# bg5sbk/dragonboat

Hardware: AMD Instinct MI355X
Metric: quorum-commit decisions/sec (whole node) + % HBM roofline at 1/2/4/8 GPUs (higher is better)
Workload: dtype u64

## Files before the change

### dragonboat_amd/csrc/hq_commit_body.h

```cpp
#pragma once

#include <type_traits>

#include "hq_internal.h"

namespace {

typedef uint64_t u64x2 __attribute__((ext_vector_type(2)));
typedef uint32_t u32x4 __attribute__((ext_vector_type(4)));

__device__ __forceinline__ u64x2 ld_stream2(const uint64_t *p) {
    return __builtin_nontemporal_load(reinterpret_cast<const u64x2 *>(p));
}
__device__ __forceinline__ void st_stream2(uint64_t *p, u64x2 v) {
    *reinterpret_cast<u64x2 *>(p) = v;
}

struct CommitK {
    uint64_t G;
    uint64_t stride;
    const uint64_t *match;
    const uint64_t *cin;
    uint64_t *cout;
    const uint64_t *last;
    const void *aux;
    const void *ring;
    uint64_t *changed, *fallback;
    const uint8_t *nv;
    uint32_t R, reserved;
};
static_assert(sizeof(CommitK) == 96, "keep the decision kernels' argument at 96 bytes");

__device__ __forceinline__ void ce(uint64_t &a, uint64_t &b) {
    const uint64_t lo = a < b ? a : b;
    const uint64_t hi = a < b ? b : a;
    a = lo;
    b = hi;
}

template <int N>
__device__ __forceinline__ void sort_net(uint64_t (&v)[N]) {
#pragma unroll
    for (int r = 0; r < N; ++r) {
#pragma unroll
        for (int i = r & 1; i + 1 < N; i += 2) ce(v[i], v[i + 1]);
    }
}

template <int N>
__device__ __forceinline__ uint64_t quorum_match_uniform(uint64_t (&v)[N]) {
    if constexpr (N == 1) {
        return v[0];
    } else if constexpr (N == 2) {
        return v[0] < v[1] ? v[0] : v[1];
    } else if constexpr (N == 3) {
        ce(v[0], v[1]);
        ce(v[1], v[2]);
        return v[0] > v[1] ? v[0] : v[1];
    } else {
        sort_net<N>(v);
        return v[N - (N / 2 + 1)];
    }
}

template <int N>
__device__ __forceinline__ uint64_t quorum_match_pern(uint64_t (&v)[N], int n) {
    sort_net<N>(v);
    const int idx = N - (n / 2 + 1);
    uint64_t r = 0;
#pragma unroll
    for (int k = 0; k < N; ++k) r = (k == idx) ? v[k] : r;
    return r;
}

__device__ __forceinline__ uint64_t spread32(uint32_t x) {
    uint64_t v = x;
    v = (v | (v << 16)) & 0x0000FFFF0000FFFFull;
    v = (v | (v << 8)) & 0x00FF00FF00FF00FFull;
    v = (v | (v << 4)) & 0x0F0F0F0F0F0F0F0Full;
    v = (v | (v << 2)) & 0x3333333333333333ull;
    v = (v | (v << 1)) & 0x5555555555555555ull;
    return v;
}

template <int N, int FORM, bool PERN>
__device__ __forceinline__ void decide(const CommitK &a, uint64_t g, uint64_t (&m)[N], int n,
                                       uint64_t cin, uint64_t last, uint64_t aux,
                                       uint64_t &cout, bool &chg, bool &fb) {
    cout = cin;
    chg = false;
    fb = false;
    if constexpr (PERN) {
        if (n < 1 || n > N) {
            fb = true;
            return;
        }
#pragma unroll
        for (int s = 0; s < N; ++s) m[s] = (s < n) ? m[s] : 0;
    }
    uint64_t q;
    if constexpr (PERN) {
        q = quorum_match_pern<N>(m, n);
    } else {
        q = quorum_match_uniform<N>(m);
    }
    if constexpr (FORM == HQ_FORM_TERM_START) {
        chg = (q > cin) & (q >= aux) & (q <= last);
    } else if constexpr (FORM == HQ_FORM_TERM_MASK) {
        fb = (cin > last) || (last - cin > a.R);
        chg = !fb && q > cin && q <= last && ((aux >> (q & (uint64_t)(a.R - 1))) & 1);
    } else if constexpr (FORM == HQ_FORM_TERM_RING32) {
        fb = (aux == 0) | (aux >= 0xFFFFFFFFull) | (cin > last) || (last - cin > a.R);
        if (!fb && q > cin && q <= last) {
            const uint32_t lterm = static_cast<const uint32_t *>(a.ring)[g * a.R + (q & (uint64_t)(a.R - 1))];
            chg = lterm == (uint32_t)aux;
        }
    } else {
        fb = (aux == 0) | (cin > last) || (last - cin > a.R);
        if (!fb && q > cin && q <= last) {
            const uint64_t lterm = static_cast<const uint64_t *>(a.ring)[g * a.R + (q & (uint64_t)(a.R - 1))];
            chg = lterm == aux;
        }
    }
    cout = chg ? q : cin;
}

#ifndef HQ_TILE_SCHED_BARRIER
#define HQ_TILE_SCHED_BARRIER 1
#endif

template <bool WT>
__device__ __forceinline__ void st8(uint64_t *p, uint64_t v) {
    if constexpr (WT) __hip_atomic_store(p, v, __ATOMIC_RELAXED, __HIP_MEMORY_SCOPE_AGENT);
    else *p = v;
}

template <class T>
__device__ __forceinline__ T *byte_off(T *p, uint32_t off) {
    return reinterpret_cast<T *>(reinterpret_cast<
        typename std::conditional<std::is_const<T>::value, const char, char>::type *>(p) + off);
}

template <int N, int FORM, bool PERN, int LEAD, bool INPLACE, bool WT = false, bool SOFF = false>
__device__ __forceinline__ void commit_tile(const CommitK &a, uint64_t wbase, uint64_t lane) {
    constexpr uint64_t T = HQ_TILE_GROUPS, H = T / 2;
    constexpr int NR = N - LEAD;
    const uint64_t *t = a.match + (wbase / T) * a.stride + lane * 2;
    const uint64_t ga = wbase + lane, gb = ga + H;
    bool ca = false, cb = false, fa = false, fb = false;
    if (wbase + T <= a.G) {
        const uint64_t *tb = a.match + (wbase / T) * a.stride;
        const uint32_t lo = (uint32_t)lane * 16u;
        auto row = [&](int r) -> const uint64_t * {
            if constexpr (SOFF) return byte_off(tb + r * T, lo);
            return t + r * T;
        };
        uint64_t m0[N], m1[N];
#pragma unroll
        for (int s = LEAD; s < N; ++s) {
            const u64x2 v = ld_stream2(row(s - LEAD));
            m0[s] = v.x;
            m1[s] = v.y;
        }
        const u64x2 ci = ld_stream2(row(NR)), la = ld_stream2(row(NR + 1));
        if constexpr (LEAD) {
            m0[0] = la.x;
            m1[0] = la.y;
        }
        u64x2 ax;
        if constexpr (FORM == HQ_FORM_TERM_MASK) {
            const uint32_t *mp =
                SOFF ? byte_off(reinterpret_cast<const uint32_t *>(tb + (NR + 2) * T), lo / 4)
                     : reinterpret_cast<const uint32_t *>(
                           reinterpret_cast<const uint16_t *>(t - lane * 2 + (NR + 2) * T) + lane * 2);
            const uint32_t mm = __builtin_nontemporal_load(mp);
            ax = (u64x2){mm & 0xFFFFu, mm >> 16};
        } else {
            ax = ld_stream2(row(NR + 2));
        }
#if HQ_TILE_SCHED_BARRIER
        if constexpr (N <= 5) __builtin_amdgcn_sched_barrier(0);
#endif
        const int na = PERN ? (int)a.nv[ga] : N, nb = PERN ? (int)a.nv[gb] : N;
        uint64_t coa, cob;
#ifdef HQ_TILE_COPY
        coa = ci.x ^ la.x ^ ax.x;
        cob = ci.y ^ la.y ^ ax.y;
#pragma unroll
        for (int s = LEAD; s < N; ++s) {
            coa ^= m0[s];
            cob ^= m1[s];
        }
        ca = coa & 1;
        cb = cob & 1;
        (void)na;
        (void)nb;
#else
        decide<N, FORM, PERN>(a, ga, m0, na, ci.x, la.x, ax.x, coa, ca, fa);
        decide<N, FORM, PERN>(a, gb, m1, nb, ci.y, la.y, ax.y, cob, cb, fb);
#endif
        if constexpr (INPLACE) {
            uint64_t *cr = const_cast<uint64_t *>(row(NR));
            if constexpr (WT) {
                st8<true>(cr, coa);
                st8<true>(cr + 1, cob);
            } else {
                st_stream2(cr, (u64x2){coa, cob});
            }
        } else if constexpr (SOFF) {
            uint64_t *cb0 = a.cout + wbase;
            st8<WT>(byte_off(cb0, lo / 2), coa);
            st8<WT>(byte_off(cb0 + H, lo / 2), cob);
        } else {
            st8<WT>(a.cout + ga, coa);
            st8<WT>(a.cout + gb, cob);
        }
    } else {
        auto single = [&](int j, bool &c, bool &f) {
            const uint64_t g = ga + H * j;
            uint64_t m[N];
            const uint64_t last = t[(NR + 1) * T + j];
#pragma unroll
            for (int s = LEAD; s < N; ++s) m[s] = t[(s - LEAD) * T + j];
            if constexpr (LEAD) m[0] = last;
            const uint64_t ax =
                FORM == HQ_FORM_TERM_MASK
                    ? (uint64_t)reinterpret_cast<const uint16_t *>(t - lane * 2 + (NR + 2) * T)[lane * 2 + j]
                    : t[(NR + 2) * T + j];
            uint64_t co;
            decide<N, FORM, PERN>(a, g, m, PERN ? (int)a.nv[g] : N, t[NR * T + j], last, ax,
                                  co, c, f);
            if constexpr (INPLACE) st8<WT>(const_cast<uint64_t *>(t) + NR * T + j, co);
            else st8<WT>(a.cout + g, co);
        };
        if (ga < a.G) single(0, ca, fa);
        if (gb < a.G) single(1, cb, fb);
    }
    const uint64_t ba = __ballot(ca), bb = __ballot(cb);
    const uint64_t xa = __ballot(fa), xb = __ballot(fb);
    const uint64_t w = (wbase >> 6) + lane;
    if (lane < 2 && w < ((a.G + 63) >> 6)) {
        if (a.changed) st8<WT>(a.changed + w, lane ? bb : ba);
        if (a.fallback) st8<WT>(a.fallback + w, lane ? xb : xa);
    }
}

}
```

### dragonboat_amd/csrc/hq_engine.hip

```cpp
#include <algorithm>
#include <chrono>
#include <cstdlib>
#include <cstring>
#include <mutex>
#include <new>
#include <string>
#include <thread>

#include "hq_commit_body.h"

namespace {

constexpr uint32_t kEngineMaxDepth = 64;
constexpr uint64_t kDescStop = 1;
constexpr int kShards = 8;
constexpr int kPollCopies = 16;
constexpr int kPollStride = 32;
constexpr int kInit = 32;

struct EngineDesc {
    uint64_t G;
    const uint64_t *tiles;
    uint64_t *cout;
    uint64_t *changed;
    uint64_t *fallback;
    uint64_t seq;
    uint64_t flags;
    uint64_t per;
};
static_assert(sizeof(EngineDesc) == 64, "a descriptor is 8 relay lanes of u64");

struct EngineK {
    uint64_t stride;
    uint64_t idle_ticks;
    uint32_t R;
    uint32_t depth;
    uint32_t signal;
    uint32_t epoch;
    const uint64_t *h_posted;
    uint64_t *h_done;
    uint64_t *h_clock;
    const EngineDesc *h_ring;
    uint64_t *d_posted;
    uint64_t *d_arrive;
    uint64_t *d_top;
    uint64_t *d_cursor;
    EngineDesc *d_ring;
    uint64_t *d_polled;
    uint64_t *d_exit;
    uint64_t init_base;
    uint32_t init_count, pad;
    EngineDesc init[kInit];
};

__device__ __forceinline__ uint64_t uniform64(uint64_t v) {
    const uint32_t lo = __builtin_amdgcn_readfirstlane((uint32_t)v);
    const uint32_t hi = __builtin_amdgcn_readfirstlane((uint32_t)(v >> 32));
    return ((uint64_t)hi << 32) | lo;
}

__device__ __forceinline__ uint64_t now_ticks() { return __builtin_amdgcn_s_memrealtime(); }

template <class T>
__device__ __forceinline__ T *as_global(uint64_t v) {
    typedef __attribute__((address_space(1))) T GT;
    return (T *)(GT *)v;
}

typedef __attribute__((address_space(1))) const volatile EngineK GlobalEngineK;
__device__ __forceinline__ GlobalEngineK &kargs() {
    return *(GlobalEngineK *)reinterpret_cast<uintptr_t>(__builtin_amdgcn_kernarg_segment_ptr());
}

template <class T>
__device__ __forceinline__ T *gp(T *p) { return as_global<T>(reinterpret_cast<uint64_t>(p)); }

__device__ void relay(GlobalEngineK &e, uint32_t lane) {
    const uint64_t have = __hip_atomic_load(gp(e.d_posted), __ATOMIC_RELAXED, __HIP_MEMORY_SCOPE_AGENT);
    const uint64_t hp = __hip_atomic_load(gp(e.h_posted), __ATOMIC_RELAXED, __HIP_MEMORY_SCOPE_SYSTEM);
    if (hp <= have) return;
    __builtin_amdgcn_fence(__ATOMIC_ACQUIRE, "");
    const uint64_t n = hp - have < e.depth ? hp - have : e.depth;
    const uint64_t dmask = e.depth - 1;
    for (uint64_t base = 0; base < n; base += 32) {
        uint64_t v[4];
#pragma unroll
        for (int j = 0; j < 4; ++j) {
            const uint64_t i = base + (lane >> 3) + 8 * j;
            v[j] = i < n ? __hip_atomic_load(
                               reinterpret_cast<const uint64_t *>(gp(e.h_ring) + ((have + i) & dmask)) +
                                   (lane & 7),
                               __ATOMIC_RELAXED, __HIP_MEMORY_SCOPE_SYSTEM)
                         : 0;
        }
#pragma unroll
        for (int j = 0; j < 4; ++j) {
            const uint64_t i = base + (lane >> 3) + 8 * j;
            if (i < n)
                __hip_atomic_store(reinterpret_cast<uint64_t *>(gp(e.d_ring) + ((have + i) & dmask)) +
                                       (lane & 7),
                                   v[j], __ATOMIC_RELAXED, __HIP_MEMORY_SCOPE_AGENT);
        }
    }
    __builtin_amdgcn_fence(__ATOMIC_RELEASE, "agent");
    if (lane == 0)
        __hip_atomic_store(gp(e.d_posted), have + n, __ATOMIC_RELAXED, __HIP_MEMORY_SCOPE_AGENT);
    if (lane < (uint32_t)kPollCopies)
        __hip_atomic_store(gp(e.d_polled) + lane * kPollStride, have + n, __ATOMIC_RELAXED,
                           __HIP_MEMORY_SCOPE_AGENT);
}

__device__ void arrive(GlobalEngineK &e, uint64_t s) {
    const uint64_t slot = s & (e.depth - 1);
    const uint32_t shard = blockIdx.x % kShards;
    const uint32_t nshard = gridDim.x < (uint32_t)kShards ? gridDim.x : (uint32_t)kShards;
    const uint64_t per = (gridDim.x - shard + kShards - 1) / kShards;
    uint64_t *ctr = gp(e.d_arrive) + slot * kShards + shard;
    if (__hip_atomic_fetch_add(ctr, (uint64_t)1, __ATOMIC_RELAXED, __HIP_MEMORY_SCOPE_AGENT) + 1 !=
        per)
        return;
    __hip_atomic_store(ctr, (uint64_t)0, __ATOMIC_RELAXED, __HIP_MEMORY_SCOPE_AGENT);
    if (__hip_atomic_fetch_add(gp(e.d_top) + slot, (uint64_t)1, __ATOMIC_RELAXED,
                               __HIP_MEMORY_SCOPE_AGENT) + 1 != nshard)
        return;
    __hip_atomic_store(gp(e.d_top) + slot, (uint64_t)0, __ATOMIC_RELAXED, __HIP_MEMORY_SCOPE_AGENT);
    __hip_atomic_store(gp(e.h_clock) + slot, now_ticks(), __ATOMIC_RELAXED, __HIP_MEMORY_SCOPE_SYSTEM);
    __hip_atomic_store(gp(e.h_done) + slot, s + 1, __ATOMIC_RELEASE, __HIP_MEMORY_SCOPE_SYSTEM);
}

struct EngineLds {
    EngineDesc ring[kEngineMaxDepth];
    uint32_t end[kEngineMaxDepth];
    uint32_t fin[kEngineMaxDepth];
    uint32_t tgt[kEngineMaxDepth];
    uint64_t known;
    uint32_t ticket;
    uint32_t top_end;
    uint32_t done;
    uint32_t waiting, lock, exit;
};

__device__ __forceinline__ bool before(uint32_t a, uint32_t b) { return (int32_t)(a - b) < 0; }

__device__ __forceinline__ uint64_t wg_len(uint64_t G, uint64_t per) {
    const uint64_t tiles = (G + HQ_TILE_GROUPS - 1) / HQ_TILE_GROUPS;
    const uint64_t b0 = (uint64_t)blockIdx.x * per;
    return b0 >= tiles ? 0 : (tiles - b0 < per ? tiles - b0 : per);
}

__device__ void install(GlobalEngineK &e, EngineLds &l, uint64_t from, uint64_t to) {
    const uint64_t dmask = e.depth - 1;
    uint32_t top = l.top_end;
    for (uint64_t s = from; s < to; ++s) {
        const EngineDesc &d = l.ring[s & dmask];
        const uint32_t len = (d.flags & kDescStop) ? 0u : (uint32_t)wg_len(d.G, d.per);
        top += len;
        l.end[s & dmask] = top;
        l.tgt[s & dmask] += len;
        if (len == 0 && e.signal && !(d.flags & kDescStop)) arrive(e, s);
    }
    l.top_end = top;
}

__device__ __forceinline__ uint64_t lds_known(EngineLds &l) {
    return __hip_atomic_load(&l.known, __ATOMIC_ACQUIRE, __HIP_MEMORY_SCOPE_WORKGROUP);
}

__device__ __forceinline__ uint32_t wave_u32(uint32_t v) { return __builtin_amdgcn_readfirstlane(v); }

__device__ __forceinline__ uint64_t polled(GlobalEngineK &e) {
    return uniform64(__hip_atomic_load(gp(e.d_polled) + (blockIdx.x % kPollCopies) * kPollStride,
                                       __ATOMIC_RELAXED, __HIP_MEMORY_SCOPE_AGENT));
}

__device__ __forceinline__ void pull(GlobalEngineK &e, EngineLds &l, uint64_t from, uint64_t p,
                                     uint32_t lane) {
    __builtin_amdgcn_fence(__ATOMIC_ACQUIRE, "agent");
    const uint64_t dmask = e.depth - 1;
    for (uint64_t i = lane >> 3; i < p - from; i += 8) {
        const uint64_t slot = (from + i) & dmask;
        reinterpret_cast<uint64_t *>(l.ring + slot)[lane & 7] = __hip_atomic_load(
            reinterpret_cast<const uint64_t *>(gp(e.d_ring) + slot) + (lane & 7),
            __ATOMIC_RELAXED, __HIP_MEMORY_SCOPE_AGENT);
    }
    if (lane == 0) {
        install(e, l, from, p);
        __hip_atomic_store(&l.known, p, __ATOMIC_RELEASE, __HIP_MEMORY_SCOPE_WORKGROUP);
    }
}

template <int WPW>
__device__ uint64_t frontier(GlobalEngineK &e, EngineLds &l, uint64_t s, uint32_t lane) {
    uint64_t k = lds_known(l);
    if (k > s) return k;
    const bool relayer = blockIdx.x == 0;
    if (lane == 0) __hip_atomic_fetch_add(&l.waiting, 1u, __ATOMIC_RELAXED, __HIP_MEMORY_SCOPE_WORKGROUP);
    for (;;) {
        k = uniform64(lds_known(l));
        if (k > s) break;
        if (wave_u32(__hip_atomic_load(&l.exit, __ATOMIC_RELAXED, __HIP_MEMORY_SCOPE_WORKGROUP)))
            return s;
        uint32_t got = 0;
        if (lane == 0)
            got = __hip_atomic_exchange(&l.lock, 1u, __ATOMIC_ACQUIRE, __HIP_MEMORY_SCOPE_WORKGROUP) == 0;
        if (wave_u32(got)) {
            k = uniform64(lds_known(l));
            if (k > s) {
                if (lane == 0) __hip_atomic_store(&l.lock, 0u, __ATOMIC_RELEASE, __HIP_MEMORY_SCOPE_WORKGROUP);
                break;
            }
            const uint64_t t0 = now_ticks();
            uint32_t backoff = 1;
            bool leave = false;
            for (;;) {
                if (relayer) relay(e, lane);
                const uint64_t p = polled(e);
                if (p > s) {
                    pull(e, l, s, p, lane);
                    k = p;
                    break;
                }
                const bool all_waiting =
                    wave_u32(__hip_atomic_load(&l.waiting, __ATOMIC_RELAXED,
                                               __HIP_MEMORY_SCOPE_WORKGROUP)) == (uint32_t)WPW;
                if (relayer) {
                    if (all_waiting && now_ticks() - t0 > e.idle_ticks) {
                        __builtin_amdgcn_fence(__ATOMIC_RELEASE, "agent");
                        if (lane == 0)
                            __hip_atomic_store(gp(e.d_exit), (uint64_t)e.epoch, __ATOMIC_RELAXED,
                                               __HIP_MEMORY_SCOPE_AGENT);
                        leave = true;
                    }
                } else if (all_waiting) {
                    const bool ended = uniform64(__hip_atomic_load(gp(e.d_exit), __ATOMIC_RELAXED,
                                                                   __HIP_MEMORY_SCOPE_AGENT)) == e.epoch;
                    __builtin_amdgcn_fence(__ATOMIC_ACQUIRE, "agent");
                    const uint64_t p2 = polled(e);
                    if ((ended && p2 <= s) || now_ticks() - t0 > 64 * e.idle_ticks) leave = true;
                }
                if (leave) {
                    if (lane == 0)
                        __hip_atomic_store(&l.exit, 1u, __ATOMIC_RELAXED, __HIP_MEMORY_SCOPE_WORKGROUP);
                    k = s;
                    break;
                }
                for (uint32_t i = 0; i < backoff; ++i) __builtin_amdgcn_s_sleep(16);
                backoff = backoff < 4 ? 2 * backoff : 4;
            }
            if (lane == 0) __hip_atomic_store(&l.lock, 0u, __ATOMIC_RELEASE, __HIP_MEMORY_SCOPE_WORKGROUP);
            if (k == s) return s;
            break;
        }
        __builtin_amdgcn_s_sleep(4);
    }
    if (lane == 0) __hip_atomic_fetch_sub(&l.waiting, 1u, __ATOMIC_RELAXED, __HIP_MEMORY_SCOPE_WORKGROUP);
    return k;
}

__device__ void refresh(GlobalEngineK &e, EngineLds &l, uint64_t s, uint32_t lane) {
    if (uniform64(lds_known(l)) > s + 1) return;
    uint32_t got = 0;
    if (lane == 0)
        got = __hip_atomic_exchange(&l.lock, 1u, __ATOMIC_ACQUIRE, __HIP_MEMORY_SCOPE_WORKGROUP) == 0;
    if (!wave_u32(got)) return;
    const uint64_t k = uniform64(lds_known(l));
    if (blockIdx.x == 0) relay(e, lane);
    const uint64_t p = polled(e);
    if (p > k) pull(e, l, k, p, lane);
    if (lane == 0) __hip_atomic_store(&l.lock, 0u, __ATOMIC_RELEASE, __HIP_MEMORY_SCOPE_WORKGROUP);
}

__device__ __forceinline__ uint32_t claim(EngineLds &l, uint32_t lane) {
    uint32_t t = 0;
    if (lane == 0) t = __hip_atomic_fetch_add(&l.ticket, 1u, __ATOMIC_RELAXED, __HIP_MEMORY_SCOPE_WORKGROUP);
    return wave_u32(t);
}

#ifdef HQ_ENGINE_WGPROF
constexpr uint32_t kWgProfMax = 2048;
__device__ uint64_t g_wgprof[kWgProfMax * 8];
#endif

template <int N, int FORM, int LEAD, bool INPLACE, int BLK, bool SIG>
__global__ __launch_bounds__(BLK) __attribute__((amdgpu_waves_per_eu(BLK >= 1024 ? 8 : 1, 8)))
void k_commit_engine(const EngineK e) {
    constexpr int WPW = BLK / 64;
    __shared__ EngineLds l;
    const uint32_t lane = threadIdx.x & 63;
    const uint32_t wv = __builtin_amdgcn_readfirstlane(threadIdx.x >> 6);
    const uint64_t dmask = e.depth - 1;
    const uint64_t s0 = uniform64(gp(e.d_cursor)[blockIdx.x]);
    for (uint32_t i = threadIdx.x; i < kEngineMaxDepth; i += BLK) {
        l.fin[i] = 0;
        l.tgt[i] = 0;
    }
    for (uint32_t i = threadIdx.x; i < e.init_count * 8; i += BLK)
        reinterpret_cast<uint64_t *>(l.ring + ((e.init_base + (i >> 3)) & dmask))[i & 7] =
            reinterpret_cast<const uint64_t *>(e.init)[i];
    __syncthreads();
    if (threadIdx.x == 0) {
        const uint64_t top = e.init_base + e.init_count;
        l.ticket = 0;
        l.done = 0;
        l.top_end = 0;
        l.waiting = l.lock = l.exit = 0;
        if (top > s0) install(kargs(), l, s0, top);
        l.known = top > s0 ? top : s0;
    }
    __syncthreads();
    if (blockIdx.x == 0 && wv == 0) refresh(kargs(), l, s0, lane);
    uint64_t s = s0;
    uint64_t known = s0;
    uint32_t e_prev = 0;
#ifdef HQ_ENGINE_WGPROF
    uint64_t *const prof = blockIdx.x < kWgProfMax ? g_wgprof + (size_t)blockIdx.x * 8 : nullptr;
    uint64_t p_busy = 0, p_tiles = 0, p_front = 0, p_nfront = 0, p_refr = 0;
    if (prof && threadIdx.x == 0) {
        __hip_atomic_store(prof + 0, now_ticks(), __ATOMIC_RELAXED, __HIP_MEMORY_SCOPE_AGENT);
        __hip_atomic_store(prof + 1, (uint64_t)__builtin_amdgcn_s_getreg((3 << 11) | 20),
                           __ATOMIC_RELAXED, __HIP_MEMORY_SCOPE_AGENT);
        __hip_atomic_store(prof + 2, (uint64_t)__builtin_amdgcn_s_getreg((31 << 11) | 4),
                           __ATOMIC_RELAXED, __HIP_MEMORY_SCOPE_AGENT);
    }
#endif
    uint32_t t = claim(l, lane);
    bool pend = false;
    uint64_t p_s = 0;
    uint32_t p_tgt = 0;
    auto count = [&]() {
        if constexpr (INPLACE) {
            if (lane == 0)
                __hip_atomic_fetch_add(&l.done, 1u, __ATOMIC_RELEASE, __HIP_MEMORY_SCOPE_WORKGROUP);
        }
        if constexpr (SIG) {
            uint32_t f = 0;
            if (lane == 0)
                f = __hip_atomic_fetch_add(&l.fin[p_s & dmask], 1u, __ATOMIC_RELAXED,
                                           __HIP_MEMORY_SCOPE_WORKGROUP) + 1;
            if (wave_u32(f) == p_tgt && lane == 0) arrive(kargs(), p_s);
        }
        pend = false;
    };
    auto drain = [&]() {
        if constexpr (SIG || INPLACE) {
            if (pend) {
                asm volatile("s_waitcnt vmcnt(0)" ::: "memory");
                count();
            }
        }
    };
    for (;;) {
        if (s >= known) {
            drain();
            #ifdef HQ_ENGINE_WGPROF
            const uint64_t p_f0 = now_ticks();
            #endif
            known = frontier<WPW>(kargs(), l, s, lane);
            #ifdef HQ_ENGINE_WGPROF
            p_front += now_ticks() - p_f0;
            ++p_nfront;
            #endif
            if (known <= s) break;
        }
        const uint64_t slot = s & dmask;
        const uint64_t *d = reinterpret_cast<const uint64_t *>(l.ring + slot);
        if (uniform64(d[6]) & kDescStop) {
            drain();
            if (t == e_prev && lane == 0) arrive(kargs(), s);
            ++s;
            break;
        }
        const uint32_t e_cur = wave_u32(l.end[slot]);
        if (before(t, e_cur)) {
            CommitK k{};
            k.stride = e.stride;
            k.R = e.R;
            k.G = uniform64(d[0]);
            k.match = as_global<const uint64_t>(uniform64(d[1]));
            k.cout = as_global<uint64_t>(uniform64(d[2]));
            k.changed = as_global<uint64_t>(uniform64(d[3]));
            k.fallback = as_global<uint64_t>(uniform64(d[4]));
            const uint64_t b0 = (uint64_t)blockIdx.x * uniform64(d[7]);
            uint32_t tgt = 0;
            if constexpr (SIG) tgt = wave_u32(l.tgt[slot]);
            if constexpr (INPLACE) {
                drain();
                while (before(wave_u32(__hip_atomic_load(&l.done, __ATOMIC_ACQUIRE,
                                                         __HIP_MEMORY_SCOPE_WORKGROUP)),
                              e_prev))
                    __builtin_amdgcn_s_sleep(2);
            }
#ifdef HQ_ENGINE_WGPROF
            const uint64_t p_t0 = now_ticks();
#endif
            do {
                const uint64_t wbase = uniform64((b0 + (uint32_t)(t - e_prev)) * HQ_TILE_GROUPS);
                uint32_t ln;
                asm volatile("v_mov_b32 %0, %1" : "=v"(ln) : "v"(lane));
                commit_tile<N, FORM, false, LEAD, INPLACE, SIG, true>(k, wbase, ln);
                if constexpr (SIG || INPLACE) {
                    asm volatile("" ::: "memory");
                    if (pend) count();
                    pend = true;
                    p_s = s;
                    p_tgt = tgt;
                }
#ifdef HQ_ENGINE_WGPROF
                ++p_tiles;
#endif
                t = claim(l, lane);
            } while (before(t, e_cur));
#ifdef HQ_ENGINE_WGPROF
            p_busy += now_ticks() - p_t0;
#endif
        }
        e_prev = e_cur;
        ++s;
        #ifdef HQ_ENGINE_WGPROF
        const uint64_t p_r0 = now_ticks();
        #endif
        if (wv == 0) refresh(kargs(), l, s, lane);
        #ifdef HQ_ENGINE_WGPROF
        if (wv == 0) p_refr += now_ticks() - p_r0;
        #endif
    }
    drain();
    if (lane == 0 && wv == 0) gp(e.d_cursor)[blockIdx.x] = s;
#ifdef HQ_ENGINE_WGPROF
    if (prof && lane == 0) {
        __hip_atomic_fetch_add(prof + 3, p_busy, __ATOMIC_RELAXED, __HIP_MEMORY_SCOPE_AGENT);
        __hip_atomic_fetch_add(prof + 4, p_tiles, __ATOMIC_RELAXED, __HIP_MEMORY_SCOPE_AGENT);
        __hip_atomic_fetch_max(prof + 5, now_ticks(), __ATOMIC_RELAXED, __HIP_MEMORY_SCOPE_AGENT);
        __hip_atomic_fetch_add(prof + 6, p_front | (p_nfront << 40), __ATOMIC_RELAXED,
                               __HIP_MEMORY_SCOPE_AGENT);
        __hip_atomic_fetch_add(prof + 7, p_refr, __ATOMIC_RELAXED, __HIP_MEMORY_SCOPE_AGENT);
    }
#endif
}

typedef void (*EngineKernel)(const EngineK);

template <int N, int FORM, int LEAD, bool INPLACE>
void engine_kernel_for(bool sig, EngineKernel *fn, int *blk) {
    constexpr int B = N <= 5 ? 1024 : 512;
    *fn = sig ? k_commit_engine<N, FORM, LEAD, INPLACE, B, true>
              : k_commit_engine<N, FORM, LEAD, INPLACE, B, false>;
    *blk = B;
}

template <int N>
int engine_kernel_n(uint32_t form, uint32_t layout, bool sig, EngineKernel *fn, int *blk) {
    const bool lead = (layout & 0xFFu) == HQ_LAYOUT_TILES_LEADER;
    const bool inplace = (layout & HQ_LAYOUT_IN_PLACE) != 0;
#define HQ_ENGINE_PICK(F)                                                                        \
    if (inplace) engine_kernel_for<N, F, 1, true>(sig, fn, blk);                                 \
    else if (lead) engine_kernel_for<N, F, 1, false>(sig, fn, blk);                              \
    else engine_kernel_for<N, F, 0, false>(sig, fn, blk);
    if (form == HQ_FORM_TERM_MASK) {
        HQ_ENGINE_PICK(HQ_FORM_TERM_MASK)
    } else {
        HQ_ENGINE_PICK(HQ_FORM_TERM_START)
    }
#undef HQ_ENGINE_PICK
    return HQ_OK;
}

int engine_kernel(uint32_t n, uint32_t form, uint32_t layout, bool sig, EngineKernel *fn, int *blk) {
    switch (n) {
    case 1: return engine_kernel_n<1>(form, layout, sig, fn, blk);
    case 2: return engine_kernel_n<2>(form, layout, sig, fn, blk);
    case 3: return engine_kernel_n<3>(form, layout, sig, fn, blk);
    case 4: return engine_kernel_n<4>(form, layout, sig, fn, blk);
    case 5: return engine_kernel_n<5>(form, layout, sig, fn, blk);
    case 6: return engine_kernel_n<6>(form, layout, sig, fn, blk);
    case 7: return engine_kernel_n<7>(form, layout, sig, fn, blk);
    default: return engine_kernel_n<8>(form, layout, sig, fn, blk);
    }
}

}

struct hq_engine {
    hq_ctx *ctx = nullptr;
    std::mutex mu;
    std::string err;
    hq_engine_config cfg{};
    hipStream_t stream = nullptr;
    hipEvent_t ev_start = nullptr, ev_end = nullptr;
    EngineKernel fn = nullptr;
    int block = 0;
    uint32_t grid = 0;
    EngineK k{};
    char *host = nullptr;
    char *dev = nullptr;
    uint64_t posted = 0;
    uint64_t completed = 0;
    bool running = false;
    uint64_t launches = 0;
    double launch_ms = 0.0;
    uint64_t relaunches = 0;
    uint32_t epoch = 0;
    uint64_t wait_limit_ms = 60000;
    size_t cur_off = 0, exit_off = 0, polled_off = 0;
    uint64_t inplace_G = 0;
};

namespace {

int efail(hq_engine *e, int code, const std::string &msg) {
    e->err = msg;
    return code;
}

int echeck(hq_engine *e, hipError_t r, const char *what) {
    if (r == hipSuccess) return HQ_OK;
    return efail(e, r == hipErrorOutOfMemory ? HQ_E_NOMEM : HQ_E_DEVICE,
                 std::string(what) + ": " + hipGetErrorString(r));
}

uint64_t host_load(const uint64_t *p) { return __atomic_load_n(p, __ATOMIC_ACQUIRE); }

int fold_if_ended(hq_engine *e, bool *ended) {
    *ended = !e->running;
    if (!e->running) return HQ_OK;
    const hipError_t q = hipEventQuery(e->ev_end);
    if (q == hipErrorNotReady) return HQ_OK;
    int rc = echeck(e, q, "hipEventQuery(engine)");
    if (rc) return rc;
    float ms = 0.f;
    rc = echeck(e, hipEventElapsedTime(&ms, e->ev_start, e->ev_end), "hipEventElapsedTime");
    if (rc) return rc;
    e->launches++;
    e->launch_ms += ms;
    e->running = false;
    *ended = true;
    return HQ_OK;
}

int launch(hq_engine *e) {
    const EngineDesc *ring = reinterpret_cast<const EngineDesc *>(e->host + 128 + 16 * (size_t)e->cfg.depth);
    const uint64_t n = std::min<uint64_t>(e->posted - e->completed, kInit);
    e->k.init_base = e->completed;
    e->k.init_count = (uint32_t)n;
    for (uint64_t i = 0; i < n; ++i) e->k.init[i] = ring[(e->completed + i) & (e->cfg.depth - 1)];
    e->k.epoch = ++e->epoch;
    int rc = echeck(e, hipSetDevice(e->ctx->device), "hipSetDevice");
    if (!rc) rc = echeck(e, hipEventRecord(e->ev_start, e->stream), "hipEventRecord");
    if (rc) return rc;
    hipLaunchKernelGGL(e->fn, dim3(e->grid), dim3(e->block), 0, e->stream, e->k);
    rc = echeck(e, hipGetLastError(), "k_commit_engine");
    if (!rc) rc = echeck(e, hipEventRecord(e->ev_end, e->stream), "hipEventRecord");
    if (rc) return rc;
    e->running = true;
    return HQ_OK;
}

int ensure_running(hq_engine *e) {
    bool ended = false;
    int rc = fold_if_ended(e, &ended);
    if (rc || !ended) return rc;
    return launch(e);
}

uint64_t *done_arr(hq_engine *e) { return reinterpret_cast<uint64_t *>(e->host + 128); }

bool step_done(hq_engine *e, uint64_t seq) {
    return host_load(done_arr(e) + (seq & (e->cfg.depth - 1))) >= seq + 1;
}

int wait_step(hq_engine *e, uint64_t seq) {
    const auto t0 = std::chrono::steady_clock::now();
    uint32_t spins = 0;
    for (;;) {
        if (step_done(e, seq)) break;
        bool ended = false;
        int rc = fold_if_ended(e, &ended);
        if (rc) return rc;
        if (ended) {
            if (step_done(e, seq)) break;
            e->relaunches++;
            rc = launch(e);
            if (rc) return rc;
        }
        if (++spins > 256) {
            std::this_thread::yield();
            spins = 0;
            if (std::chrono::steady_clock::now() - t0 > std::chrono::milliseconds(e->wait_limit_ms))
                return efail(e, HQ_E_DEVICE, "hq_engine: step " + std::to_string(seq) +
                                                 " not completed within the wait limit (" +
                                                 std::to_string(e->wait_limit_ms) + " ms)");
        }
    }
    while (e->completed < e->posted && step_done(e, e->completed)) e->completed++;
    return HQ_OK;
}

int write_desc(hq_engine *e, const EngineDesc &d) {
    EngineDesc *ring = reinterpret_cast<EngineDesc *>(e->host + 128 + 16 * (size_t)e->cfg.depth);
    std::memcpy(ring + (e->posted & (e->cfg.depth - 1)), &d, sizeof d);
    e->posted++;
    __atomic_store_n(reinterpret_cast<uint64_t *>(e->host), e->posted, __ATOMIC_RELEASE);
    return HQ_OK;
}

int drain_locked(hq_engine *e);

int make_room(hq_engine *e) {
    if (e->posted - e->completed < e->cfg.depth) return HQ_OK;
    if (e->cfg.flags & HQ_ENGINE_SIGNAL) {
        int rc = ensure_running(e);
        if (!rc) rc = wait_step(e, e->completed);
        return rc;
    }
    return drain_locked(e);
}

int drain_locked(hq_engine *e) {
    bool ended = false;
    int rc = fold_if_ended(e, &ended);
    if (rc) return rc;
    if (!ended) {
        if (e->posted - e->completed >= e->cfg.depth) {
            if (!(e->cfg.flags & HQ_ENGINE_SIGNAL)) {
                return efail(e, HQ_E_STATE, "hq_engine: ring full without a STOP slot");
            }
            rc = wait_step(e, e->completed);
            if (rc) return rc;
        }
        EngineDesc d{};
        d.flags = kDescStop;
        d.seq = e->posted;
        const uint64_t seq = e->posted;
        write_desc(e, d);
        rc = wait_step(e, seq);
        if (rc) return rc;
        rc = echeck(e, hipEventSynchronize(e->ev_end), "hipEventSynchronize(engine)");
        if (rc) return rc;
        rc = fold_if_ended(e, &ended);
        if (rc) return rc;
    } else if (e->posted != e->completed) {
        EngineDesc d{};
        d.flags = kDescStop;
        d.seq = e->posted;
        const uint64_t seq = e->posted;
        write_desc(e, d);
        rc = launch(e);
        if (!rc) rc = wait_step(e, seq);
        if (!rc) rc = echeck(e, hipEventSynchronize(e->ev_end), "hipEventSynchronize(engine)");
        if (!rc) rc = fold_if_ended(e, &ended);
        if (rc) return rc;
    }
    e->completed = e->posted;
    return HQ_OK;
}

int validate_post(hq_engine *e, const hq_commit_args *a) {
    const hq_engine_config &c = e->cfg;
    if (a->n_max != c.n_max || a->form != c.form || a->layout != c.layout)
        return efail(e, HQ_E_INVAL, "hq_engine_post: n_max / form / layout differ from the engine's");
    if (a->n_voting)
        return efail(e, HQ_E_INVAL, "hq_engine_post: per-group n is not served (bucket by n)");
    if (c.form == HQ_FORM_TERM_MASK && a->ring_len != c.ring_len)
        return efail(e, HQ_E_INVAL, "hq_engine_post: ring_len differs from the engine's");
    if (a->G == 0) return HQ_OK;
    const bool in_place = (c.layout & HQ_LAYOUT_IN_PLACE) != 0;
    if (!a->match || (!in_place && !a->committed_out))
        return efail(e, HQ_E_INVAL, "hq_engine_post: NULL tiles (match) / committed_out");
    if (!hq::aligned16(a->match) || (!in_place && !hq::aligned16(a->committed_out)))
        return efail(e, HQ_E_INVAL, "hq_engine_post: tiles and committed_out must be 16-byte aligned");
    if (in_place && e->inplace_G && a->G != e->inplace_G)
        return efail(e, HQ_E_INVAL, "hq_engine_post: an in-place table's steps must keep one G (the "
                                    "engine's first in-place post set it)");
    return HQ_OK;
}

}

extern "C" {

int hq_engine_open(hq_ctx *ctx, const hq_engine_config *cfg, hq_engine **out) {
    if (!ctx || !cfg || !out) return HQ_E_INVAL;
    *out = nullptr;
    hq_engine_config c = *cfg;
    if (c.depth == 0) c.depth = kEngineMaxDepth;
    if (c.idle_us == 0) c.idle_us = 1000;
    if (c.n_max < 1 || c.n_max > HQ_MAX_VOTERS)
        return hq::fail(ctx, HQ_E_INVAL, "hq_engine_open: n_max must be 1..8");
    if (c.form != HQ_FORM_TERM_START && c.form != HQ_FORM_TERM_MASK)
        return hq::fail(ctx, HQ_E_INVAL, "hq_engine_open: the engine serves the term-start and "
                                         "term-mask forms");
    if (c.layout != HQ_LAYOUT_TILES && c.layout != HQ_LAYOUT_TILES_LEADER &&
        c.layout != (HQ_LAYOUT_TILES_LEADER | HQ_LAYOUT_IN_PLACE))
        return hq::fail(ctx, HQ_E_INVAL, "hq_engine_open: layout must be HQ_LAYOUT_TILES, "
                                         "_TILES_LEADER or _TILES_LEADER | HQ_LAYOUT_IN_PLACE");
    if (c.layout == HQ_LAYOUT_TILES_LEADER && c.n_max < 1)
        return hq::fail(ctx, HQ_E_INVAL, "hq_engine_open: bad n_max");
    if (c.form == HQ_FORM_TERM_MASK &&
        (c.ring_len < 1 || c.ring_len > 16 || (c.ring_len & (c.ring_len - 1))))
        return hq::fail(ctx, HQ_E_INVAL, "hq_engine_open: mask form needs ring_len <= 16 (power of two)");
    if (c.depth < 2 || c.depth > kEngineMaxDepth || (c.depth & (c.depth - 1)))
        return hq::fail(ctx, HQ_E_INVAL, "hq_engine_open: depth must be a power of two in 2..64");
    if (c.flags & ~(uint32_t)HQ_ENGINE_SIGNAL)
        return hq::fail(ctx, HQ_E_INVAL, "hq_engine_open: unknown flags");
    hq_engine *e = new (std::nothrow) hq_engine();
    if (!e) return hq::fail(ctx, HQ_E_NOMEM, "hq_engine_open: out of host memory");
    e->ctx = ctx;
    e->cfg = c;
    engine_kernel(c.n_max, c.form, c.layout, (c.flags & HQ_ENGINE_SIGNAL) != 0, &e->fn, &e->block);
    int rc = hq::check_hip(ctx, hipSetDevice(ctx->device), "hipSetDevice");
    int cus = 0, per_cu = 0;
    if (!rc) rc = hq::check_hip(ctx, hipDeviceGetAttribute(&cus, hipDeviceAttributeMultiprocessorCount,
                                                           ctx->device), "hipDeviceGetAttribute");
    if (!rc) rc = hq::check_hip(ctx, hipOccupancyMaxActiveBlocksPerMultiprocessor(
                                         &per_cu, reinterpret_cast<const void *>(e->fn), e->block, 0),
                                "hipOccupancyMaxActiveBlocksPerMultiprocessor");
    if (!rc && (cus < 1 || per_cu < 1))
        rc = hq::fail(ctx, HQ_E_DEVICE, "hq_engine_open: the engine kernel does not fit a CU");
    if (rc) {
        delete e;
        return rc;
    }
    e->grid = (uint32_t)(cus * per_cu);
    if (c.max_workgroups && c.max_workgroups < e->grid) e->grid = c.max_workgroups;
    const size_t D = c.depth;
    const size_t host_bytes = 128 + 16 * D + sizeof(EngineDesc) * D;
    if (const char *w = std::getenv("HQ_ENGINE_WAIT_MS")) e->wait_limit_ms = std::max(1, std::atoi(w));
    const size_t arrive_off = 128, top_off = arrive_off + 8 * kShards * D, cur_off = top_off + 8 * D;
    const size_t ring_off = (cur_off + 8 * (size_t)e->grid + 127) & ~(size_t)127;
    const size_t exit_off = ring_off + sizeof(EngineDesc) * D;
    const size_t polled_off = exit_off + 256;
    const size_t dev_bytes = polled_off + 8 * kPollCopies * kPollStride;
    e->cur_off = cur_off;
    e->exit_off = exit_off;
    e->polled_off = polled_off;
    void *hp = nullptr, *dp = nullptr;
    rc = hq::check_hip(ctx, hipStreamCreateWithFlags(&e->stream, hipStreamNonBlocking),
                       "hipStreamCreateWithFlags");
    if (!rc) rc = hq::check_hip(ctx, hipEventCreate(&e->ev_start), "hipEventCreate");
    if (!rc) rc = hq::check_hip(ctx, hipEventCreate(&e->ev_end), "hipEventCreate");
    if (!rc) rc = hq::check_hip(ctx, hipHostMalloc(&hp, host_bytes, hipHostMallocCoherent),
                                "hipHostMalloc(engine ring)");
    if (!rc) rc = hq::check_hip(ctx, hipMalloc(&dp, dev_bytes), "hipMalloc(engine)");
    if (!rc) rc = hq::check_hip(ctx, hipMemset(dp, 0, dev_bytes), "hipMemset(engine)");
    e->host = static_cast<char *>(hp);
    e->dev = static_cast<char *>(dp);
    if (rc) {
        hq_engine_close(e);
        return rc;
    }
    std::memset(hp, 0, host_bytes);
    EngineK &k = e->k;
    k.stride = hq_commit_tile_words_for(c.n_max, c.form, c.layout);
    k.idle_ticks = (uint64_t)c.idle_us * 100;
    k.R = c.form == HQ_FORM_TERM_MASK ? c.ring_len : 16;
    k.depth = c.depth;
    k.signal = (c.flags & HQ_ENGINE_SIGNAL) ? 1u : 0u;
    k.h_posted = reinterpret_cast<const uint64_t *>(e->host);
    k.h_done = reinterpret_cast<uint64_t *>(e->host + 128);
    k.h_clock = reinterpret_cast<uint64_t *>(e->host + 128 + 8 * D);
    k.h_ring = reinterpret_cast<const EngineDesc *>(e->host + 128 + 16 * D);
    k.d_posted = reinterpret_cast<uint64_t *>(e->dev);
    k.d_arrive = reinterpret_cast<uint64_t *>(e->dev + arrive_off);
    k.d_top = reinterpret_cast<uint64_t *>(e->dev + top_off);
    k.d_cursor = reinterpret_cast<uint64_t *>(e->dev + cur_off);
    k.d_ring = reinterpret_cast<EngineDesc *>(e->dev + ring_off);
    k.d_polled = reinterpret_cast<uint64_t *>(e->dev + polled_off);
    k.d_exit = reinterpret_cast<uint64_t *>(e->dev + exit_off);
    *out = e;
    return HQ_OK;
}

namespace {

int post_locked(hq_engine *e, const hq_commit_args *args, uint32_t count, uint64_t *first_seq,
                bool start) {
    if (count && !args) return efail(e, HQ_E_INVAL, "hq_engine_post: args is NULL");
    const uint64_t keep_G = e->inplace_G;
    for (uint32_t i = 0; i < count; ++i) {
        int rc = validate_post(e, args + i);
        if (!rc && (e->cfg.layout & HQ_LAYOUT_IN_PLACE) && args[i].G) e->inplace_G = args[i].G;
        if (rc) {
            e->inplace_G = keep_G;
            return rc;
        }
    }
    e->inplace_G = keep_G;
    if (first_seq) *first_seq = e->posted;
    int rc = echeck(e, hipSetDevice(e->ctx->device), "hipSetDevice");
    for (uint32_t i = 0; i < count && !rc; ++i) {
        const bool signal = (e->cfg.flags & HQ_ENGINE_SIGNAL) != 0;
        if (!signal && e->posted - e->completed >= e->cfg.depth - 1) rc = drain_locked(e);
        else rc = make_room(e);
        if (rc) break;
        EngineDesc d{};
        d.G = args[i].G;
        d.tiles = args[i].match;
        d.cout = args[i].committed_out;
        d.changed = args[i].changed;
        d.fallback = args[i].fallback;
        d.seq = e->posted;
        const uint64_t tiles = (d.G + HQ_TILE_GROUPS - 1) / HQ_TILE_GROUPS;
        d.per = (tiles + e->grid - 1) / e->grid;
        if ((e->cfg.layout & HQ_LAYOUT_IN_PLACE) && d.G) e->inplace_G = d.G;
        rc = write_desc(e, d);
    }
    if (!rc && count && start) rc = ensure_running(e);
    return rc;
}

}

int hq_engine_post(hq_engine *e, const hq_commit_args *args, uint32_t count, uint64_t *first_seq) {
    if (!e) return HQ_E_INVAL;
    std::lock_guard<std::mutex> g(e->mu);
    return post_locked(e, args, count, first_seq, true);
}

int hq_engine_run(hq_engine *e, const hq_commit_args *args, uint32_t count, uint64_t *first_seq) {
    if (!e) return HQ_E_INVAL;
    std::lock_guard<std::mutex> g(e->mu);
    int rc = post_locked(e, args, count, first_seq, false);
    if (!rc) rc = echeck(e, hipSetDevice(e->ctx->device), "hipSetDevice");
    return rc ? rc : drain_locked(e);
}

int hq_engine_wait(hq_engine *e, uint64_t seq) {
    if (!e) return HQ_E_INVAL;
    std::lock_guard<std::mutex> g(e->mu);
    if (seq >= e->posted) return efail(e, HQ_E_INVAL, "hq_engine_wait: step not posted");
    if (seq < e->completed) return HQ_OK;
    if (!(e->cfg.flags & HQ_ENGINE_SIGNAL)) return drain_locked(e);
    int rc = echeck(e, hipSetDevice(e->ctx->device), "hipSetDevice");
    if (!rc) rc = ensure_running(e);
    if (!rc) rc = wait_step(e, seq);
    return rc;
}

int hq_engine_drain(hq_engine *e) {
    if (!e) return HQ_E_INVAL;
    std::lock_guard<std::mutex> g(e->mu);
    int rc = echeck(e, hipSetDevice(e->ctx->device), "hipSetDevice");
    return rc ? rc : drain_locked(e);
}

int hq_engine_timing(hq_engine *e, uint64_t *launches, double *total_ms, int reset) {
    if (!e) return HQ_E_INVAL;
    std::lock_guard<std::mutex> g(e->mu);
    bool ended = false;
    int rc = fold_if_ended(e, &ended);
    if (rc) return rc;
    if (launches) *launches = e->launches;
    if (total_ms) *total_ms = e->launch_ms;
    if (reset) {
        e->launches = 0;
        e->launch_ms = 0.0;
    }
    return HQ_OK;
}

int hq_engine_info(hq_engine *e, hq_engine_stats *out) {
    if (!e || !out) return HQ_E_INVAL;
    std::lock_guard<std::mutex> g(e->mu);
    out->grid = e->grid;
    out->block = (uint32_t)e->block;
    out->posted = e->posted;
    out->completed = e->completed;
    out->relaunches = e->relaunches;
    out->running = e->running ? 1u : 0u;
    out->depth = e->cfg.depth;
    return HQ_OK;
}

int hq_engine_done_clock(hq_engine *e, uint64_t seq, uint64_t *ticks) {
    if (!e || !ticks) return HQ_E_INVAL;
    std::lock_guard<std::mutex> g(e->mu);
    if (!(e->cfg.flags & HQ_ENGINE_SIGNAL))
        return efail(e, HQ_E_STATE, "hq_engine_done_clock: needs HQ_ENGINE_SIGNAL");
    if (seq >= e->posted || !step_done(e, seq) ||
        host_load(done_arr(e) + (seq & (e->cfg.depth - 1))) != seq + 1)
        return efail(e, HQ_E_STATE, "hq_engine_done_clock: step not complete or slot reused");
    *ticks = host_load(done_arr(e) + e->cfg.depth + (seq & (e->cfg.depth - 1)));
    return HQ_OK;
}

int hq_engine_dump(hq_engine *e, uint64_t *out, uint32_t n_words) {
    if (!e || !out) return HQ_E_INVAL;
    std::lock_guard<std::mutex> g(e->mu);
    const uint32_t head = 8;
    const size_t D = e->cfg.depth;
    if (n_words < head + e->grid + (kShards + 1) * D)
        return efail(e, HQ_E_INVAL, "hq_engine_dump: needs 8 + grid + 9 * depth words");
    hipStream_t st = nullptr;
    int rc = echeck(e, hipSetDevice(e->ctx->device), "hipSetDevice");
    if (!rc) rc = echeck(e, hipStreamCreateWithFlags(&st, hipStreamNonBlocking), "hipStreamCreate");
    uint64_t dp = 0, polled = 0, ex = 0;
    if (!rc) rc = echeck(e, hipMemcpyAsync(&dp, e->dev, 8, hipMemcpyDeviceToHost, st), "hipMemcpyAsync");
    if (!rc) rc = echeck(e, hipMemcpyAsync(&polled, e->dev + e->polled_off, 8, hipMemcpyDeviceToHost, st), "hipMemcpyAsync");
    if (!rc) rc = echeck(e, hipMemcpyAsync(&ex, e->dev + e->exit_off, 8, hipMemcpyDeviceToHost, st), "hipMemcpyAsync");
    if (!rc) rc = echeck(e, hipMemcpyAsync(out + head, e->dev + e->cur_off, 8 * (size_t)e->grid,
                                           hipMemcpyDeviceToHost, st), "hipMemcpyAsync");
    if (!rc) rc = echeck(e, hipMemcpyAsync(out + head + e->grid, e->dev + 128,
                                           8 * (kShards + 1) * D, hipMemcpyDeviceToHost, st),
                         "hipMemcpyAsync");
    if (!rc) rc = echeck(e, hipStreamSynchronize(st), "hipStreamSynchronize");
    if (st) (void)hipStreamDestroy(st);
    if (rc) return rc;
    out[0] = host_load(reinterpret_cast<const uint64_t *>(e->host));
    out[1] = dp;
    out[2] = polled;
    out[3] = ex;
    out[4] = e->epoch;
    out[5] = e->grid;
    out[6] = e->completed;
    out[7] = e->running ? 1 : 0;
    return HQ_OK;
}

const char *hq_engine_last_error(const hq_engine *e) { return e ? e->err.c_str() : ""; }

#ifdef HQ_ENGINE_WGPROF
int hq_engine_wgprof(uint64_t *out, uint32_t n_words, int reset) {
    const size_t bytes = sizeof(uint64_t) * 8 * kWgProfMax;
    if (out && n_words < 8 * kWgProfMax) return HQ_E_INVAL;
    if (hipDeviceSynchronize() != hipSuccess) return HQ_E_DEVICE;
    if (out && hipMemcpyFromSymbol(out, HIP_SYMBOL(g_wgprof), bytes) != hipSuccess) return HQ_E_DEVICE;
    if (reset) {
        void *z = nullptr;
        if (hipGetSymbolAddress(&z, HIP_SYMBOL(g_wgprof)) != hipSuccess ||
            hipMemset(z, 0, bytes) != hipSuccess || hipDeviceSynchronize() != hipSuccess)
            return HQ_E_DEVICE;
    }
    return HQ_OK;
}
#endif

void hq_engine_close(hq_engine *e) {
    if (!e) return;
    (void)hipSetDevice(e->ctx->device);
    if (e->host && e->dev && e->stream) {
        std::lock_guard<std::mutex> g(e->mu);
        (void)drain_locked(e);
    }
    if (e->stream) (void)hipStreamSynchronize(e->stream);
    if (e->ev_start) (void)hipEventDestroy(e->ev_start);
    if (e->ev_end) (void)hipEventDestroy(e->ev_end);
    if (e->host) (void)hipHostFree(e->host);
    if (e->dev) (void)hipFree(e->dev);
    if (e->stream) (void)hipStreamDestroy(e->stream);
    delete e;
}

}
```

Baseline: 110.4 billion.

## Overlap tile loads with next-ticket claim and cross steps without leaving tile loop

Splits commit_tile into a load-issue phase and a finish phase so the persistent engine can issue a tile's global loads, then claim the next ticket and resolve step boundaries while those loads are in flight. The inner loop now advances across descriptor steps directly, fetching the next step's G/match/base and running the in-place barrier and refresh only when needed, instead of falling back to the outer loop per step. The signal path reads the target from LDS at count time rather than caching it per step. This adds complexity in step and state tracking (s, e_prev, known) and raises register pressure from holding the tile rows across the claim.

```diff
diff --git a/dragonboat_amd/csrc/hq_commit_body.h b/dragonboat_amd/csrc/hq_commit_body.h
--- a/dragonboat_amd/csrc/hq_commit_body.h
+++ b/dragonboat_amd/csrc/hq_commit_body.h
@@ -141,46 +141,72 @@
         typename std::conditional<std::is_const<T>::value, const char, char>::type *>(p) + off);
 }
 
-template <int N, int FORM, bool PERN, int LEAD, bool INPLACE, bool WT = false, bool SOFF = false>
-__device__ __forceinline__ void commit_tile(const CommitK &a, uint64_t wbase, uint64_t lane) {
+template <int N>
+struct TileRows {
+    uint64_t m0[N], m1[N];
+    u64x2 ci, la, ax;
+    uint32_t mm;
+};
+
+template <int N, int FORM, int LEAD, bool SOFF>
+__device__ __forceinline__ void tile_loads(const uint64_t *t, const uint64_t *tb, uint32_t lo,
+                                           uint64_t lane, TileRows<N> &r) {
+    constexpr uint64_t T = HQ_TILE_GROUPS;
+    constexpr int NR = N - LEAD;
+    auto row = [&](int i) -> const uint64_t * {
+        if constexpr (SOFF) return byte_off(tb + i * T, lo);
+        return t + i * T;
+    };
+#pragma unroll
+    for (int s = LEAD; s < N; ++s) {
+        const u64x2 v = ld_stream2(row(s - LEAD));
+        r.m0[s] = v.x;
+        r.m1[s] = v.y;
+    }
+    r.ci = ld_stream2(row(NR));
+    r.la = ld_stream2(row(NR + 1));
+    if constexpr (LEAD) {
+        r.m0[0] = r.la.x;
+        r.m1[0] = r.la.y;
+    }
+    if constexpr (FORM == HQ_FORM_TERM_MASK) {
+        const uint32_t *mp =
+            SOFF ? byte_off(reinterpret_cast<const uint32_t *>(tb + (NR + 2) * T), lo / 4)
+                 : reinterpret_cast<const uint32_t *>(
+                       reinterpret_cast<const uint16_t *>(t - lane * 2 + (NR + 2) * T) + lane * 2);
+        r.mm = __builtin_nontemporal_load(mp);
+        r.ax = (u64x2){r.mm & 0xFFFFu, r.mm >> 16};
+    } else {
+        r.ax = ld_stream2(row(NR + 2));
+    }
+#if HQ_TILE_SCHED_BARRIER
+    if constexpr (N <= 5) __builtin_amdgcn_sched_barrier(0);
+#endif
+}
+
+template <int N, int FORM, int LEAD, bool SOFF>
+__device__ __forceinline__ void tile_issue(const CommitK &a, uint64_t wbase, uint64_t lane,
+                                           TileRows<N> &r) {
+    const uint64_t *tb = a.match + (wbase / HQ_TILE_GROUPS) * a.stride;
+    tile_loads<N, FORM, LEAD, SOFF>(tb + lane * 2, tb, (uint32_t)lane * 16u, lane, r);
+}
+
+template <int N, int FORM, bool PERN, int LEAD, bool INPLACE, bool WT, bool SOFF, bool ISSUE = false>
+__device__ __forceinline__ void tile_finish(const CommitK &a, uint64_t wbase, uint64_t lane,
+                                            TileRows<N> &r, bool full) {
     constexpr uint64_t T = HQ_TILE_GROUPS, H = T / 2;
     constexpr int NR = N - LEAD;
     const uint64_t *t = a.match + (wbase / T) * a.stride + lane * 2;
     const uint64_t ga = wbase + lane, gb = ga + H;
     bool ca = false, cb = false, fa = false, fb = false;
-    if (wbase + T <= a.G) {
+    if (ISSUE ? wbase + T <= a.G : full) {
         const uint64_t *tb = a.match + (wbase / T) * a.stride;
         const uint32_t lo = (uint32_t)lane * 16u;
-        auto row = [&](int r) -> const uint64_t * {
-            if constexpr (SOFF) return byte_off(tb + r * T, lo);
-            return t + r * T;
-        };
-        uint64_t m0[N], m1[N];
-#pragma unroll
-        for (int s = LEAD; s < N; ++s) {
-            const u64x2 v = ld_stream2(row(s - LEAD));
-            m0[s] = v.x;
-            m1[s] = v.y;
-        }
-        const u64x2 ci = ld_stream2(row(NR)), la = ld_stream2(row(NR + 1));
-        if constexpr (LEAD) {
-            m0[0] = la.x;
-            m1[0] = la.y;
-        }
-        u64x2 ax;
-        if constexpr (FORM == HQ_FORM_TERM_MASK) {
-            const uint32_t *mp =
-                SOFF ? byte_off(reinterpret_cast<const uint32_t *>(tb + (NR + 2) * T), lo / 4)
-                     : reinterpret_cast<const uint32_t *>(
-                           reinterpret_cast<const uint16_t *>(t - lane * 2 + (NR + 2) * T) + lane * 2);
-            const uint32_t mm = __builtin_nontemporal_load(mp);
-            ax = (u64x2){mm & 0xFFFFu, mm >> 16};
-        } else {
-            ax = ld_stream2(row(NR + 2));
-        }
-#if HQ_TILE_SCHED_BARRIER
-        if constexpr (N <= 5) __builtin_amdgcn_sched_barrier(0);
-#endif
+        if constexpr (ISSUE) tile_loads<N, FORM, LEAD, SOFF>(t, tb, lo, lane, r);
+        uint64_t (&m0)[N] = r.m0, (&m1)[N] = r.m1;
+        const u64x2 ci = r.ci, la = r.la;
+        u64x2 ax = r.ax;
+        if constexpr (FORM == HQ_FORM_TERM_MASK && !ISSUE) ax = (u64x2){r.mm & 0xFFFFu, r.mm >> 16};
         const int na = PERN ? (int)a.nv[ga] : N, nb = PERN ? (int)a.nv[gb] : N;
         uint64_t coa, cob;
 #ifdef HQ_TILE_COPY
@@ -200,7 +226,7 @@
         decide<N, FORM, PERN>(a, gb, m1, nb, ci.y, la.y, ax.y, cob, cb, fb);
 #endif
         if constexpr (INPLACE) {
-            uint64_t *cr = const_cast<uint64_t *>(row(NR));
+            uint64_t *cr = const_cast<uint64_t *>(SOFF ? byte_off(tb + NR * T, lo) : t + NR * T);
             if constexpr (WT) {
                 st8<true>(cr, coa);
                 st8<true>(cr + 1, cob);
@@ -245,4 +271,10 @@
     }
 }
 
-}
+template <int N, int FORM, bool PERN, int LEAD, bool INPLACE, bool WT = false, bool SOFF = false>
+__device__ __forceinline__ void commit_tile(const CommitK &a, uint64_t wbase, uint64_t lane) {
+    TileRows<N> r;
+    tile_finish<N, FORM, PERN, LEAD, INPLACE, WT, SOFF, true>(a, wbase, lane, r, true);
+}
+
+}
diff --git a/dragonboat_amd/csrc/hq_engine.hip b/dragonboat_amd/csrc/hq_engine.hip
--- a/dragonboat_amd/csrc/hq_engine.hip
+++ b/dragonboat_amd/csrc/hq_engine.hip
@@ -288,7 +288,7 @@
     __shared__ EngineLds l;
     const uint32_t lane = threadIdx.x & 63;
     const uint32_t wv = __builtin_amdgcn_readfirstlane(threadIdx.x >> 6);
-    const uint64_t dmask = e.depth - 1;
+    const uint32_t dmask = e.depth - 1;
     const uint64_t s0 = uniform64(gp(e.d_cursor)[blockIdx.x]);
     for (uint32_t i = threadIdx.x; i < kEngineMaxDepth; i += BLK) {
         l.fin[i] = 0;
@@ -326,18 +326,16 @@
     uint32_t t = claim(l, lane);
     bool pend = false;
     uint64_t p_s = 0;
-    uint32_t p_tgt = 0;
     auto count = [&]() {
         if constexpr (INPLACE) {
             if (lane == 0)
                 __hip_atomic_fetch_add(&l.done, 1u, __ATOMIC_RELEASE, __HIP_MEMORY_SCOPE_WORKGROUP);
         }
         if constexpr (SIG) {
-            uint32_t f = 0;
-            if (lane == 0)
-                f = __hip_atomic_fetch_add(&l.fin[p_s & dmask], 1u, __ATOMIC_RELAXED,
-                                           __HIP_MEMORY_SCOPE_WORKGROUP) + 1;
-            if (wave_u32(f) == p_tgt && lane == 0) arrive(kargs(), p_s);
+            if (lane == 0 &&
+                __hip_atomic_fetch_add(&l.fin[p_s & dmask], 1u, __ATOMIC_RELAXED,
+                                       __HIP_MEMORY_SCOPE_WORKGROUP) + 1 == l.tgt[p_s & dmask])
+                arrive(kargs(), p_s);
         }
         pend = false;
     };
@@ -349,13 +347,25 @@
             }
         }
     };
+    auto step_in = [&](uint64_t slot, uint64_t &G, const uint64_t *&match, uint64_t &b0) {
+        const uint64_t *d = reinterpret_cast<const uint64_t *>(l.ring + slot);
+        G = uniform64(d[0]);
+        match = as_global<const uint64_t>(uniform64(d[1]));
+        b0 = (uint64_t)blockIdx.x * uniform64(d[7]);
+    };
+    auto step_out = [&](uint64_t slot, CommitK &k) {
+        const uint64_t *d = reinterpret_cast<const uint64_t *>(l.ring + slot);
+        k.cout = as_global<uint64_t>(uniform64(d[2]));
+        k.changed = as_global<uint64_t>(uniform64(d[3]));
+        k.fallback = as_global<uint64_t>(uniform64(d[4]));
+    };
     for (;;) {
         if (s >= known) {
             drain();
             #ifdef HQ_ENGINE_WGPROF
             const uint64_t p_f0 = now_ticks();
             #endif
-            known = frontier<WPW>(kargs(), l, s, lane);
+            known = uniform64(frontier<WPW>(kargs(), l, s, lane));
             #ifdef HQ_ENGINE_WGPROF
             p_front += now_ticks() - p_f0;
             ++p_nfront;
@@ -363,56 +373,102 @@
             if (known <= s) break;
         }
         const uint64_t slot = s & dmask;
-        const uint64_t *d = reinterpret_cast<const uint64_t *>(l.ring + slot);
-        if (uniform64(d[6]) & kDescStop) {
+        if (uniform64(reinterpret_cast<const uint64_t *>(l.ring + slot)[6]) & kDescStop) {
             drain();
             if (t == e_prev && lane == 0) arrive(kargs(), s);
             ++s;
             break;
         }
-        const uint32_t e_cur = wave_u32(l.end[slot]);
+        uint32_t e_cur = wave_u32(l.end[slot]);
         if (before(t, e_cur)) {
             CommitK k{};
             k.stride = e.stride;
             k.R = e.R;
-            k.G = uniform64(d[0]);
-            k.match = as_global<const uint64_t>(uniform64(d[1]));
-            k.cout = as_global<uint64_t>(uniform64(d[2]));
-            k.changed = as_global<uint64_t>(uniform64(d[3]));
-            k.fallback = as_global<uint64_t>(uniform64(d[4]));
-            const uint64_t b0 = (uint64_t)blockIdx.x * uniform64(d[7]);
-            uint32_t tgt = 0;
-            if constexpr (SIG) tgt = wave_u32(l.tgt[slot]);
-            if constexpr (INPLACE) {
-                drain();
-                while (before(wave_u32(__hip_atomic_load(&l.done, __ATOMIC_ACQUIRE,
-                                                         __HIP_MEMORY_SCOPE_WORKGROUP)),
-                              e_prev))
-                    __builtin_amdgcn_s_sleep(2);
-            }
-#ifdef HQ_ENGINE_WGPROF
-            const uint64_t p_t0 = now_ticks();
-#endif
-            do {
-                const uint64_t wbase = uniform64((b0 + (uint32_t)(t - e_prev)) * HQ_TILE_GROUPS);
+            uint64_t b0;
+            step_in(slot, k.G, k.match, b0);
+            uint64_t wbase = (b0 + (uint32_t)(t - e_prev)) * HQ_TILE_GROUPS;
+            auto step_barrier = [&]() __attribute__((always_inline)) {
+                if constexpr (INPLACE) {
+                    drain();
+                    while (before(wave_u32(__hip_atomic_load(&l.done, __ATOMIC_ACQUIRE,
+                                                             __HIP_MEMORY_SCOPE_WORKGROUP)),
+                                  e_prev))
+                        __builtin_amdgcn_s_sleep(2);
+                }
+            };
+            step_barrier();
+            for (;;) {
                 uint32_t ln;
                 asm volatile("v_mov_b32 %0, %1" : "=v"(ln) : "v"(lane));
-                commit_tile<N, FORM, false, LEAD, INPLACE, SIG, true>(k, wbase, ln);
+#ifdef HQ_ENGINE_WGPROF
+                const uint64_t p_t0 = now_ticks();
+#endif
+                uint32_t t2, prev2 = e_prev, end2 = e_cur;
+                bool look = false;
+                uint64_t s2 = s, wbase2, G2 = k.G;
+                const uint64_t *match2 = k.match;
+                auto next_ticket = [&]() __attribute__((always_inline)) {
+                t2 = claim(l, lane);
+                wbase2 = wbase + (uint32_t)(t2 - t) * (uint64_t)HQ_TILE_GROUPS;
+                while (!before(t2, end2)) {
+                    prev2 = end2;
+                    ++s2;
+                    if (wv == 0 && uniform64(lds_known(l)) <= s2 + 1) look = true;
+                    if (s2 >= known) {
+                        known = uniform64(lds_known(l));
+                        if (s2 >= known) break;
+                    }
+                    const uint64_t slot2 = s2 & dmask;
+                    if (uniform64(reinterpret_cast<const uint64_t *>(l.ring + slot2)[6]) & kDescStop)
+                        break;
+                    end2 = wave_u32(l.end[slot2]);
+                    if (before(t2, end2)) {
+                        step_in(slot2, G2, match2, b0);
+                        wbase2 = (b0 + (uint32_t)(t2 - prev2)) * HQ_TILE_GROUPS;
+                    }
+                }
+                step_out(s & dmask, k);
+                };
+                TileRows<N> rows;
+                if (wbase + HQ_TILE_GROUPS <= k.G) {
+                    tile_issue<N, FORM, LEAD, true>(k, wbase, ln, rows);
+                    next_ticket();
+                    tile_finish<N, FORM, false, LEAD, INPLACE, SIG, true>(k, wbase, ln, rows, true);
+                } else {
+                    next_ticket();
+                    tile_finish<N, FORM, false, LEAD, INPLACE, SIG, true>(k, wbase, ln, rows, false);
+                }
                 if constexpr (SIG || INPLACE) {
                     asm volatile("" ::: "memory");
                     if (pend) count();
                     pend = true;
                     p_s = s;
-                    p_tgt = tgt;
                 }
 #ifdef HQ_ENGINE_WGPROF
                 ++p_tiles;
+                p_busy += now_ticks() - p_t0;
 #endif
-                t = claim(l, lane);
-            } while (before(t, e_cur));
-#ifdef HQ_ENGINE_WGPROF
-            p_busy += now_ticks() - p_t0;
-#endif
+                const bool crossed = s2 != s;
+                t = t2;
+                s = s2;
+                e_prev = prev2;
+                if (look) {
+                    #ifdef HQ_ENGINE_WGPROF
+                    const uint64_t p_r0 = now_ticks();
+                    #endif
+                    refresh(kargs(), l, s, lane);
+                    #ifdef HQ_ENGINE_WGPROF
+                    p_refr += now_ticks() - p_r0;
+                    #endif
+                }
+                if (!before(t2, end2)) break;
+                k.G = G2;
+                k.match = match2;
+                wbase = wbase2;
+                e_cur = end2;
+                if (crossed) step_barrier();
+            }
+            continue;
         }
         e_prev = e_cur;
         ++s;
@@ -425,7 +481,7 @@
         #endif
     }
     drain();
-    if (lane == 0 && wv == 0) gp(e.d_cursor)[blockIdx.x] = s;
+    if (lane == 0 && wv == 0) gp(kargs().d_cursor)[blockIdx.x] = s;
 #ifdef HQ_ENGINE_WGPROF
     if (prof && lane == 0) {
         __hip_atomic_fetch_add(prof + 3, p_busy, __ATOMIC_RELAXED, __HIP_MEMORY_SCOPE_AGENT);
```

Result: no change. 110.8 billion (median of 2 runs) (+0.3%).
